# imalexlee/simple-vk-renderer

Hardware: AMD Instinct MI355X
Metric: shaded fragments/s (higher is better)
Workload: dtype f32

## Files before the change

simple-vk-renderer_amd/csrc/k_tile.hip:

```cpp
#include <hip/hip_fp16.h>

#include <hip/hip_ext.h>

#include <cstdlib>

#include "svr_launch.h"

namespace svr {

constexpr uint32_t REC_COMMON = 0x80000000u;
#ifndef SVR_PRIO_COST
#define SVR_PRIO_COST 200u
#endif
constexpr int BATCH = 64;
constexpr uint32_t SREC = 7;

constexpr float kInv255 = 0x1.010102p-8f;
constexpr float kG0 = 0x1.c51282p-2f, kG1 = -0x1.14a3a2p-2f, kG2 = 0x1.37536ap-3f, kG3 = -0x1.778474p-5f;

__device__ __forceinline__ float lod_from_rho2(float rho2) {
  uint32_t bits = f2u(rho2);
  int e = (int)(bits >> 23) - 127;
  float m = u2f((bits & 0x7fffffu) | 0x3f800000u);
  float t = m - 1.0f;
  float g = fmaf(fmaf(fmaf(kG3, t, kG2), t, kG1), t, kG0);
  float s = t * (1.0f - t);
  float l = fmaf(s, g, t);
  float lam = 0.5f * ((float)e + l);
  lam = (rho2 <= 0x1p+100f) ? lam : 50.0f;
  lam = (rho2 >= 0x1p-100f) ? lam : -50.0f;
  return lam;
}

__device__ __forceinline__ float lerpf(float a, float b, float t) { return fmaf(t, b - a, a); }

struct TexD {
  uint32_t base_off;
  uint32_t w, h, lw, lh, levels, filters;
  float min_lod, max_lod;
};

struct Taps {
  uint32_t o00, o10, o01, o11;
  float alpha, beta;
};
template <bool POW2 = false>
__device__ __forceinline__ Taps level_taps(int wl, int hl, uint32_t base, bool linear, float u, float v) {
  float U = (u - floorf(u)) * (float)wl;
  float V = (v - floorf(v)) * (float)hl;
  float Uh = U - 0.5f, Vh = V - 0.5f;
  float fu = floorf(linear ? Uh : U), fv = floorf(linear ? Vh : V);
  Taps tp;
  tp.alpha = linear ? Uh - fu : 0.0f;
  tp.beta = linear ? Vh - fv : 0.0f;
  int i0 = (int)fu, j0 = (int)fv;
  int i1 = linear ? i0 + 1 : i0, j1 = linear ? j0 + 1 : j0;
  if (POW2) {
    i0 &= wl - 1;
    i1 &= wl - 1;
    j0 &= hl - 1;
    j1 &= hl - 1;
  } else {
    if (i0 < 0) i0 += wl;
    if (i0 >= wl) i0 -= wl;
    if (i1 >= wl) i1 -= wl;
    if (j0 < 0) j0 += hl;
    if (j0 >= hl) j0 -= hl;
    if (j1 >= hl) j1 -= hl;
  }
  const uint32_t r0 = __umul24((uint32_t)j0, (uint32_t)wl), r1 = __umul24((uint32_t)j1, (uint32_t)wl);
  tp.o00 = base + (r0 + (uint32_t)i0) * 4u;
  tp.o10 = base + (r0 + (uint32_t)i1) * 4u;
  tp.o01 = base + (r1 + (uint32_t)i0) * 4u;
  tp.o11 = base + (r1 + (uint32_t)i1) * 4u;
  return tp;
}
__device__ __forceinline__ uint32_t texel(const uint8_t* arena, uint32_t off) {
  return *reinterpret_cast<const uint32_t*>(arena + off);
}
__device__ __forceinline__ float chan(uint32_t t, int c) { return (float)((t >> (8 * c)) & 0xffu) * kInv255; }
__device__ __forceinline__ float bilerp(uint32_t t00, uint32_t t10, uint32_t t01, uint32_t t11, int c, float a, float b) {
  return lerpf(lerpf(chan(t00, c), chan(t10, c), a), lerpf(chan(t01, c), chan(t11, c), a), b);
}

__device__ __forceinline__ float interp3(float a0, float da1, float da2, float b1, float b2, float r) {
  return fmaf(b2, da2, fmaf(b1, da1, a0)) * r;
}

struct FragAttr {
  float b1, b2, r, u, v, nx, ny, nz, light, cr, cg, cb, won;
};

__device__ __forceinline__ float quad_partner_x(float v) { return u2f((uint32_t)__builtin_amdgcn_mov_dpp((int)f2u(v), 0xB1, 0xf, 0xf, true)); }
__device__ __forceinline__ float quad_partner_y(float v) { return u2f((uint32_t)__builtin_amdgcn_mov_dpp((int)f2u(v), 0x128, 0xf, 0xf, true)); }
template <bool TRACE, bool COMMON = false, bool ATTR = false>
__device__ __forceinline__ float4 shade_pixel(const FrameParams& P, uint32_t rec, int px, int py, float* trace, const bool quads = false,
                                              FragAttr* fa = nullptr) {
  const TriRec* tr = P.recs + rec;
  const uint4* q4 = reinterpret_cast<const uint4*>(tr);
  const float4* f4 = reinterpret_cast<const float4*>(tr);
  const double2* d2 = reinterpret_cast<const double2*>(tr);
  uint4 hdr = q4[0];
  float4 zrow = f4[1];
  double2 c2 = d2[2], c3 = d2[3], c4 = d2[4], c5 = d2[5], c6 = d2[6];
  uint4 td = q4[7];
  float4 s0 = f4[8], s1 = f4[9], s2 = f4[10], s3 = f4[11], s4 = f4[12], s5 = f4[13], s6 = f4[14];
  uint32_t flags = hdr.w;
  float inv_area = zrow.w;
  double A1, B1, A2, B2, e1, e2;
  double C1 = c5.y, C2 = c6.x;
  A1 = c2.y; B1 = c4.x; A2 = c3.x; B2 = c4.y;
  double dx = (double)px, dy = (double)py;
  e1 = fma(A1, dx, fma(B1, dy, C1)) + ((flags & F_T1) ? 1.0 : 0.0);
  e2 = fma(A2, dx, fma(B2, dy, C2)) + ((flags & F_T2) ? 1.0 : 0.0);
  TexD t;
  t.base_off = (uint32_t)(unsigned long long)__double_as_longlong(c6.y);
  t.w = td.x & 0xffffu;
  t.h = td.x >> 16;
  t.lw = td.y & 0xffu;
  t.lh = (td.y >> 8) & 0xffu;
  t.levels = (td.y >> 16) & 0xffu;
  t.filters = td.y >> 24;
  t.min_lod = u2f(td.z);
  t.max_lod = u2f(td.w);
  float b1 = (float)e1 * inv_area, b2 = (float)e2 * inv_area;
  float q0 = s0.x, dq1 = s0.y, dq2 = s0.z;
  const float qq = fmaf(b2, dq2, fmaf(b1, dq1, q0));
  float hb1 = 0.0f, hb2 = 0.0f, vb1 = 0.0f, vb2 = 0.0f, hq = 1.0f, vq = 1.0f;
  if (!quads) {
    double sxp = (px & 1) ? -1.0 : 1.0, syp = (py & 1) ? -1.0 : 1.0;
    hb1 = (float)fma(sxp, A1, e1) * inv_area, hb2 = (float)fma(sxp, A2, e2) * inv_area;
    vb1 = (float)fma(syp, B1, e1) * inv_area, vb2 = (float)fma(syp, B2, e2) * inv_area;
    hq = fmaf(hb2, dq2, fmaf(hb1, dq1, q0)), vq = fmaf(vb2, dq2, fmaf(vb1, dq1, q0));
  }
  float r, hr = 0.0f, vr = 0.0f;
  if (COMMON && !quads) {
    rcp3_ieee(qq, hq, vq, r, hr, vr);
  } else {
    r = rcp_ieee(qq);
  }
  const uint32_t kind = COMMON ? (uint32_t)PIPE_MESH : ((flags >> F_KIND_SHIFT) & 3u);
  float cr = interp3(s1.z, s3.z, s5.z, b1, b2, r);
  float cg = interp3(s1.w, s3.w, s5.w, b1, b2, r);
  float cb = interp3(s2.x, s4.x, s6.x, b1, b2, r);
  if (ATTR) { fa->b1 = b1; fa->b2 = b2; fa->r = r; fa->won = 1.0f; }
  if (kind == PIPE_COLORED_TRIANGLE) return make_float4(cr, cg, cb, 1.0f);
  float u = interp3(s2.y, s4.y, s6.y, b1, b2, r), v = interp3(s2.z, s4.z, s6.z, b1, b2, r);
  if (ATTR) { fa->u = u; fa->v = v; }
  if (!COMMON) {
    hr = rcp_ieee(hq);
    vr = rcp_ieee(vq);
  }
  float uh, vh, uv_, vv_;
  if (quads) {
    uh = quad_partner_x(u), vh = quad_partner_x(v);
    uv_ = quad_partner_y(u), vv_ = quad_partner_y(v);
  } else {
    uh = interp3(s2.y, s4.y, s6.y, hb1, hb2, hr), vh = interp3(s2.z, s4.z, s6.z, hb1, hb2, hr);
    uv_ = interp3(s2.y, s4.y, s6.y, vb1, vb2, vr), vv_ = interp3(s2.z, s4.z, s6.z, vb1, vb2, vr);
  }
  float dudx = (px & 1) ? (u - uh) : (uh - u);
  float dvdx = (px & 1) ? (v - vh) : (vh - v);
  float dudy = (py & 1) ? (u - uv_) : (uv_ - u);
  float dvdy = (py & 1) ? (v - vv_) : (vv_ - v);
  float W0 = (float)t.w, H0 = (float)t.h;
  float mx = dudx * W0, my = dvdx * H0;
  float nx_ = dudy * W0, ny_ = dvdy * H0;
  float rho2 = fmaxf(fmaf(mx, mx, my * my), fmaf(nx_, nx_, ny_ * ny_));
  float lambda = fminf(fmaxf(lod_from_rho2(rho2), t.min_lod), t.max_lod);
  const bool linear = COMMON ? true : (((lambda <= 0.0f) ? (t.filters & 1u) : ((t.filters >> 1) & 1u)) != 0u);
  int q = (int)t.levels - 1;
  const bool mip_linear = COMMON ? true : (((t.filters >> 2) & 1u) != 0u);
  int dn = min(max((int)ceilf(lambda + 0.5f) - 1, 0), q);
  float lc = fminf(fmaxf(lambda, 0.0f), (float)q);
  float fl = floorf(lc);
  int dhi = mip_linear ? (int)fl : dn;
  float delta = mip_linear ? lc - fl : 0.0f;
  int dlo = mip_linear ? min(dhi + 1, q) : dn;
  float us = (fabsf(u) < 8388608.0f) ? u : 0.0f, vs = (fabsf(v) < 8388608.0f) ? v : 0.0f;
  const int whi = (int)max(t.w >> dhi, 1u), hhi = (int)max(t.h >> dhi, 1u);
  const uint32_t bhi = t.base_off + mip_offset(t.lw, t.lh, (uint32_t)dhi);
  Taps th = level_taps<COMMON>(whi, hhi, bhi, linear, us, vs);
  const uint8_t* tb = P.tex_arena;
  uint32_t h00 = texel(tb, th.o00), h10 = texel(tb, th.o10), h01 = texel(tb, th.o01), h11 = texel(tb, th.o11);
  const bool two_levels = __any(delta != 0.0f);
  Taps tl = th;
  uint32_t l00 = 0, l10 = 0, l01 = 0, l11 = 0;
  if (two_levels) {
    const int wlo = (int)max(t.w >> dlo, 1u), hlo = (int)max(t.h >> dlo, 1u);
    const uint32_t step = 4u << ((uint32_t)max((int)t.lw - dhi, 0) + (uint32_t)max((int)t.lh - dhi, 0));
    const uint32_t blo = dlo != dhi ? bhi + step : bhi;
    tl = level_taps<COMMON>(wlo, hlo, blo, linear, us, vs);
    l00 = texel(tb, tl.o00);
    l10 = texel(tb, tl.o10);
    l01 = texel(tb, tl.o01);
    l11 = texel(tb, tl.o11);
  }
  float4 tx;
  tx.x = bilerp(h00, h10, h01, h11, 0, th.alpha, th.beta);
  tx.y = bilerp(h00, h10, h01, h11, 1, th.alpha, th.beta);
  tx.z = bilerp(h00, h10, h01, h11, 2, th.alpha, th.beta);
  tx.w = 1.0f;
  if (two_levels) {
    tx.x = lerpf(tx.x, bilerp(l00, l10, l01, l11, 0, tl.alpha, tl.beta), delta);
    tx.y = lerpf(tx.y, bilerp(l00, l10, l01, l11, 1, tl.alpha, tl.beta), delta);
    tx.z = lerpf(tx.z, bilerp(l00, l10, l01, l11, 2, tl.alpha, tl.beta), delta);
  }
  if (TRACE) {
    trace[0] = (float)(hdr.z >> 2); trace[1] = b1; trace[2] = b2; trace[3] = r; trace[4] = u; trace[5] = v;
    trace[6] = dudx; trace[7] = dvdx; trace[8] = dudy; trace[9] = dvdy; trace[10] = lambda;
    trace[11] = tx.x; trace[12] = tx.y; trace[13] = tx.z;
    trace[26] = hb1; trace[27] = hb2; trace[28] = vb1; trace[29] = vb2; trace[30] = hr; trace[31] = vr;
  }
  if (kind == PIPE_TEX_IMAGE) {
    tx.w = bilerp(h00, h10, h01, h11, 3, th.alpha, th.beta);
    if (two_levels) tx.w = lerpf(tx.w, bilerp(l00, l10, l01, l11, 3, tl.alpha, tl.beta), delta);
    return tx;
  }
  float nx = interp3(s0.w, s2.w, s4.w, b1, b2, r);
  float ny = interp3(s1.x, s3.x, s5.x, b1, b2, r);
  float nz = interp3(s1.y, s3.y, s5.y, b1, b2, r);
  const float* L = P.scene.sunlight_direction;
  float d = fmaf(nz, L[2], fmaf(ny, L[1], nx * L[0]));
  float light = fmaxf(d, 0.1f);
  float sunw = P.scene.sunlight_color[3];
  cr = cr * tx.x;
  cg = cg * tx.y;
  cb = cb * tx.z;
  float4 o;
  o.x = fmaf(cr * light, sunw, cr * P.scene.ambient_color[0]);
  o.y = fmaf(cg * light, sunw, cg * P.scene.ambient_color[1]);
  o.z = fmaf(cb * light, sunw, cb * P.scene.ambient_color[2]);
  o.w = 1.0f;
  if (TRACE) {
    trace[15] = nx; trace[16] = ny; trace[17] = nz; trace[18] = cr; trace[19] = cg; trace[20] = cb;
    trace[21] = light; trace[22] = o.x; trace[23] = o.y; trace[24] = o.z; trace[25] = o.w;
  }
  if (ATTR) { fa->nx = nx; fa->ny = ny; fa->nz = nz; fa->light = light; fa->cr = cr; fa->cg = cg; fa->cb = cb; }
  return o;
}

template <int FMT>
struct Codec;
template <>
struct Codec<SVR_COLOR_RGBA16F> {
  typedef uint2 enc_t;
  static __device__ __forceinline__ float pin(float x) {
    asm volatile("" : "+v"(x));
    return x;
  }
  static __device__ __forceinline__ enc_t encode(float4 c) {
    c.x = pin(c.x); c.y = pin(c.y); c.z = pin(c.z); c.w = pin(c.w);
    uint32_t r = __half_as_ushort(__float2half_rn(c.x)), g = __half_as_ushort(__float2half_rn(c.y));
    uint32_t b = __half_as_ushort(__float2half_rn(c.z)), a = __half_as_ushort(__float2half_rn(c.w));
    return make_uint2(r | (g << 16), b | (a << 16));
  }
  static __device__ __forceinline__ float4 decode(enc_t e) {
    return make_float4(__half2float(__ushort_as_half((unsigned short)(e.x & 0xffffu))),
                       __half2float(__ushort_as_half((unsigned short)(e.x >> 16))),
                       __half2float(__ushort_as_half((unsigned short)(e.y & 0xffffu))),
                       __half2float(__ushort_as_half((unsigned short)(e.y >> 16))));
  }
};
template <>
struct Codec<SVR_COLOR_RGBA8> {
  typedef uint32_t enc_t;
  static __device__ __forceinline__ uint32_t un8(float f) {
    return (uint32_t)__float2int_rn(fminf(fmaxf(f, 0.0f), 1.0f) * 255.0f);
  }
  static __device__ __forceinline__ enc_t encode(float4 c) {
    return un8(c.x) | (un8(c.y) << 8) | (un8(c.z) << 16) | (un8(c.w) << 24);
  }
  static __device__ __forceinline__ float4 decode(enc_t e) {
    return make_float4(chan(e, 0), chan(e, 1), chan(e, 2), chan(e, 3));
  }
};

template <bool INSTR, bool LIST, bool HIZ>
__device__ __forceinline__ void scan_columns(const FrameParams& P, uint4* s_cov, const uint32_t* s_list, uint32_t bin_base, uint32_t n,
                                             unsigned long long* s_depth, uint32_t* s_bm, int tx0, int ty0, int ry0, int nrows,
                                             uint32_t& n_raster, uint32_t& n_hiz_bad, uint32_t& occl) {
  auto entry = [&](uint32_t i) -> uint32_t { return LIST ? (s_list[i] & 0x7fffffffu) : P.bins[bin_base + i]; };
  const uint32_t lane = threadIdx.x & 63u, wave = threadIdx.x >> 6;
  static_assert(BATCH * 8 == 512, "two pieces per thread");
  uint4 pre0 = make_uint4(0, 0, 0, 0), pre1 = pre0;
  {
    uint32_t cnt = min((uint32_t)BATCH, n);
    const bool staged = (threadIdx.x & 7u) < SREC;
    if (staged && threadIdx.x < cnt * 8u) pre0 = reinterpret_cast<const uint4*>(P.recs + entry(threadIdx.x >> 3))[threadIdx.x & 7u];
    if (staged && threadIdx.x + 256u < cnt * 8u) pre1 = reinterpret_cast<const uint4*>(P.recs + entry(32u + (threadIdx.x >> 3)))[threadIdx.x & 7u];
  }
  constexpr uint32_t SVR_HIZ_MIN = BATCH;
  constexpr uint32_t SVR_HIZ_KEEP_COLS = 192u;
  const bool hiz = HIZ && n > (uint32_t)SVR_HIZ_MIN;
  uint32_t cur = 0, hz_cols = 0, hz_batches = 0, hz_pause = 0;
  if (hiz && threadIdx.x < 32u) s_bm[threadIdx.x] = threadIdx.x < 16u ? 0u : 0xffffffffu;
  for (uint32_t b0 = 0; b0 < n; b0 += BATCH) {
    uint32_t cnt = min((uint32_t)BATCH, n - b0);
    __syncthreads();
    const bool test = hiz && b0 && hz_pause == 0u;
    if (hiz && b0 && hz_pause) hz_pause--;
    if (test) {
      cur ^= 1u;
      const uint32_t b = threadIdx.x >> 4, k = threadIdx.x & 15u;
      const uint4* c4 = reinterpret_cast<const uint4*>(s_depth + ((b & 3u) * 8u + (k >> 1)) * TILE + (b >> 2) * 8u + (k & 1u) * 4u);
      const uint4 lo = c4[0], hi = c4[1];
      atomicMin(&s_bm[cur * 16u + b], min(min(lo.y, lo.w), min(hi.y, hi.w)));
      if (threadIdx.x < 16u) s_bm[(cur ^ 1u) * 16u + threadIdx.x] = 0xffffffffu;
    }
    if (threadIdx.x < cnt * 8u && (threadIdx.x & 7u) < SREC) s_cov[(threadIdx.x >> 3) * SREC + (threadIdx.x & 7u)] = pre0;
    if (threadIdx.x + 256u < cnt * 8u && (threadIdx.x & 7u) < SREC) s_cov[(32u + (threadIdx.x >> 3)) * SREC + (threadIdx.x & 7u)] = pre1;
    __syncthreads();
    const uint4* bm4 = reinterpret_cast<const uint4*>(s_bm + cur * 16u);
    if (b0 + BATCH < n) {
      uint32_t nb = b0 + BATCH, ncnt = min((uint32_t)BATCH, n - nb);
      const bool staged = (threadIdx.x & 7u) < SREC;
      if (staged && threadIdx.x < ncnt * 8u) pre0 = reinterpret_cast<const uint4*>(P.recs + entry(nb + (threadIdx.x >> 3)))[threadIdx.x & 7u];
      if (staged && threadIdx.x + 256u < ncnt * 8u) pre1 = reinterpret_cast<const uint4*>(P.recs + entry(nb + 32u + (threadIdx.x >> 3)))[threadIdx.x & 7u];
    }
    int cx0 = 0, cw = 0;
    bool hidden = false;
    uint32_t gone = 0;
    uint32_t zb = 0, claim = 0;
    if (lane < cnt) {
      uint4 h = s_cov[lane * SREC];
      int minx = (int)(int16_t)(h.x & 0xffffu), miny = (int)(int16_t)(h.x >> 16);
      int maxx = (int)(int16_t)(h.y & 0xffffu), maxy = (int)(int16_t)(h.y >> 16);
      cx0 = max(minx, tx0);
      const int cx1 = min(maxx, tx0 + TILE - 1);
      const int cy0 = max(miny, ry0), cy1 = min(maxy, ry0 + nrows - 1);
      cw = (cx1 >= cx0 && cy1 >= cy0) ? cx1 - cx0 + 1 : 0;
      if (HIZ && cw) {
        const float4 zr = reinterpret_cast<const float4*>(s_cov)[lane * SREC + 1u];
        const float eps = (fabsf(zr.x) + fabsf(zr.y) + fabsf(zr.z)) * 0x1p-21f;
        zb = f2u(fmaxf(fmaxf(zr.x, fmaxf(zr.x + zr.y, zr.x + zr.z)) + eps, 0.0f));
        if (minx <= tx0 && maxx >= tx0 + TILE - 1 && miny <= ry0 && maxy >= ry0 + nrows - 1) {
          const double* dd = reinterpret_cast<const double*>(s_cov + lane * SREC);
          const float x0 = (float)tx0, x1 = (float)(tx0 + TILE - 1), y0 = (float)ry0, y1 = (float)(ry0 + nrows - 1);
          bool all_in = true;
          float slack = 0.0f;
          float bc[2][4];
#pragma unroll
          for (int i = 0; i < 3; i++) {
            const float A = (float)dd[4 + i], B = (float)dd[7 + i], C = (float)dd[10 + i] + ((i == 1 && (h.w & F_T1)) || (i == 2 && (h.w & F_T2)) ? 1.0f : 0.0f);
            const float M = (fabsf(C) + fmaxf(fabsf(A * x0), fabsf(A * x1)) + fmaxf(fabsf(B * y0), fabsf(B * y1))) * 0x1p-21f;
            const float e00 = fmaf(A, x0, fmaf(B, y0, C)), e10 = fmaf(A, x1, fmaf(B, y0, C));
            const float e01 = fmaf(A, x0, fmaf(B, y1, C)), e11 = fmaf(A, x1, fmaf(B, y1, C));
            all_in = all_in && fminf(fminf(e00, e10), fminf(e01, e11)) >= M + 1.0f;
            if (i) {
              bc[i - 1][0] = e00 * zr.w; bc[i - 1][1] = e10 * zr.w; bc[i - 1][2] = e01 * zr.w; bc[i - 1][3] = e11 * zr.w;
// ... 1134 lines not shown
```

simple-vk-renderer_amd/csrc/svr_api.hip:

```cpp
#include <hip/hip_runtime.h>

#include <algorithm>
#include <chrono>
#include <cmath>
#include <cstdio>
#include <cstring>
#include <deque>
#include <memory>
#include <numeric>
#include <string>
#include <vector>

#include "../../include/svr_depth.h"
#include "../../include/svr_draw_list.h"
#include "../../include/svr_attributes.h"
#include "../../include/svr_ids.h"
#include "../../include/svr_occlusion.h"
#include "../../include/svr_views.h"
#include "svr_cull.h"
#include "svr_launch.h"

using namespace svr;

namespace {
// ... 114 lines not shown
  int fmt = SVR_COLOR_RGBA16F;
  hipStream_t stream = nullptr;
  void* color_own = nullptr;
  float* depth_own = nullptr;
  void* color = nullptr;
  float* depth = nullptr;
  uint2* ids_own = nullptr;
  uint2* ids = nullptr;
  bool ids_bound = false;
  void* attr_own[4] = {};
  void* attr[4] = {};
  bool attr_bound[4] = {};
  uint32_t sx = 0, sy = 0, sw = 0, sh = 0;
  uint32_t rstride = 1, roff = 0;
  uint32_t* present_status = nullptr;

  std::vector<MeshRes> meshes;
  std::vector<ImageRes> images;
  std::vector<SvrSamplerDesc> samplers;
  std::vector<MaterialRes> materials;
  std::vector<DrawListRes> lists;
  std::vector<std::shared_ptr<PyramidMem>> pyramids;
  uint32_t occl_bound = 0;
  SvrOcclusionStats occl_stats{};
  uint64_t mesh_epoch = 0;
  uint8_t* tex_arena = nullptr;
  size_t tex_arena_cap = 0, tex_arena_top = 0;
  std::vector<std::pair<size_t, size_t>> tex_holes;
  DevBuf tex_table;
  size_t tex_slots = 0;
  DevBuf mesh_table, mat_table;
  size_t mesh_table_n = 0, mat_table_n = 0;
  int device_flatten = 0;

  struct PassSet {
    DevBuf inputs, recs, clipq, bigq, tiles, bins, pairs, flat, sorta, occl;
    hipEvent_t ev_bin = nullptr;
    hipEvent_t ev_tile = nullptr;
    bool used = false;
  };
  static const int MAX_OPS = 8;
  static const int NSETS = 4;
  PassSet sets[NSETS];
  int set_pos = 0;
  enum class OpKind { Pass, Clear, Background, Blit, Pyramid };
  enum class PassInput { Draws, Objects, List };
  struct LoggedOp {
    OpKind kind = OpKind::Pass;
    int slot = 0;
    uint32_t seq = 0;
    bool timed = false;
    FrameParams P{};
    PassInput input = PassInput::Draws;
    bool depth_only = false;
    std::vector<DrawDesc> draws;
    std::vector<SvrRenderObject> objects;
    uint32_t n_opaque_obj = 0, n_transparent_obj = 0;
    std::shared_ptr<const ListVersion> list;
    std::vector<float> viewprojs;
    std::shared_ptr<PyramidMem> pyr;
    const float* pyr_src = nullptr;
    bool flattened() const { return input != PassInput::Draws; }
    void* target = nullptr;
    int target_fmt = 0;
    uint32_t tw = 0, th = 0, y_first = 0, n_rows = 0;
    uint64_t clear_packed = 0;
    int bg_effect = 0;
    float bg_data[16] = {};
    void* blit_dst = nullptr;
    uint32_t blit_w = 0, blit_h = 0;
    int blit_fmt = 0;
    uint32_t blit_rstride = 1, blit_roff = 0, blit_row_end = 0;
    uint32_t* blit_status = nullptr;
  };
  std::deque<LoggedOp> log;
  hipEvent_t op_done[MAX_OPS] = {};
  hipEvent_t op_start[MAX_OPS] = {};
  int op_pos = 0;
  uint32_t replayed = 0;
  struct PendingClear {
    bool valid = false;
    void* target = nullptr;
    uint32_t y0 = 0, rows = 0;
    int fmt = 0;
    uint64_t packed = 0;
  } pending_clear;
  uint32_t next_seq = 1;
  uint32_t* h_failed_seq = nullptr;
  uint32_t* d_poison = nullptr;
  hipStream_t gstream = nullptr;
  hipStream_t gstream_hi = nullptr;
  hipStream_t last_g = nullptr;
  hipEvent_t ev_gswitch = nullptr;
  DevBuf d_cvt;
  uint32_t clip_cap = 0, extra_cap = 0, bin_cap = 0;
  uint32_t debug_caps = 0;
  void* h_stage[MAX_OPS] = {};
  size_t h_stage_cap[MAX_OPS] = {};
  Counters* h_counters = nullptr;
  uint32_t* h_row_cost = nullptr;
  std::vector<uint32_t> row_cost;
  uint32_t row_cost_y0 = 0, row_cost_rows = 0;

  static const int TRING = 16;
  hipEvent_t tev[TRING][5] = {};
  bool tev_used[TRING] = {};
  bool tev_all[TRING] = {};
  int tev_pos = 0;
  int kernel_timing = 0;
  double acc_ms[3] = {0, 0, 0};
  uint32_t acc_n = 0;
  FrameParams last{};
  uint32_t last_n_draws = 0;
  bool instrument = false;
  bool tile_cycles = false;
  uint32_t tuning = 0;
  int trace_x = -1, trace_y = -1;
  DevBuf d_trace, d_tile_cycles;
  SvrStats stats{};
};

namespace {

int use_device(SvrContext* ctx) {
  HIPCHK(hipSetDevice(ctx->device));
  return SVR_OK;
}

MeshRes* get_mesh(SvrContext* ctx, SvrMesh h) {
  if (h == 0 || h > ctx->meshes.size() || !ctx->meshes[h - 1].alive) return nullptr;
  return &ctx->meshes[h - 1];
}
ImageRes* get_image(SvrContext* ctx, SvrImage h) {
  if (h == 0 || h > ctx->images.size() || !ctx->images[h - 1].alive) return nullptr;
  return &ctx->images[h - 1];
}

TexBinding make_binding(const ImageRes& im, const SvrSamplerDesc& s) {
  TexBinding tb;
  std::memset(&tb, 0, sizeof(tb));
  uint32_t filters = (uint32_t)s.mag_filter | ((uint32_t)s.min_filter << 1) | ((uint32_t)s.mipmap_mode << 2);
  tb.base_off = im.arena_off;
  tb.wh = im.w | (im.h << 16);
  tb.info = im.lw | (im.lh << 8) | (im.levels << 16) | (filters << 24);
  tb.min_lod = s.min_lod;
  tb.max_lod = s.max_lod;
  return tb;
}

int finish_pending(SvrContext* ctx);

constexpr size_t ARENA_MAX = (size_t)0xffffff00u;
constexpr size_t ARENA_ALIGN = 256;

int arena_alloc(SvrContext* ctx, size_t bytes, uint32_t* off) {
  bytes = (bytes + ARENA_ALIGN - 1) & ~(ARENA_ALIGN - 1);
  for (size_t i = 0; i < ctx->tex_holes.size(); i++) {
    auto& h = ctx->tex_holes[i];
    if (h.second >= bytes) {
      *off = (uint32_t)h.first;
      h.first += bytes;
      h.second -= bytes;
      if (h.second == 0) ctx->tex_holes.erase(ctx->tex_holes.begin() + (long)i);
      return SVR_OK;
    }
  }
  if (ctx->tex_arena_top + bytes > ARENA_MAX)
    return fail(SVR_ERR_OUT_OF_MEMORY, "svr_create_image: more than 4 GiB of texels in one context");
  if (ctx->tex_arena_top + bytes > ctx->tex_arena_cap) {
    size_t want = std::max(ctx->tex_arena_cap * 2, ctx->tex_arena_top + bytes);
    want = std::min(ARENA_MAX, (want + ((size_t)64 << 20) - 1) & ~(((size_t)64 << 20) - 1));
    if (int e = finish_pending(ctx)) return e;
    HIPCHK(hipStreamSynchronize(ctx->stream));
    uint8_t* grown = nullptr;
    HIPCHK(hipMalloc((void**)&grown, want));
    if (ctx->tex_arena_top) {
      hipError_t r = hipMemcpy(grown, ctx->tex_arena, ctx->tex_arena_top, hipMemcpyDeviceToDevice);
      if (r != hipSuccess) {
        (void)hipFree(grown);
        return fail(SVR_ERR_DEVICE, std::string("hipMemcpy(texel arena): ") + hipGetErrorString(r));
      }
    }
    if (ctx->tex_arena) (void)hipFree(ctx->tex_arena);
    ctx->tex_arena = grown;
    ctx->tex_arena_cap = want;
  }
  *off = (uint32_t)ctx->tex_arena_top;
  ctx->tex_arena_top += bytes;
  return SVR_OK;
}

void arena_free(SvrContext* ctx, size_t off, size_t bytes) {
  bytes = (bytes + ARENA_ALIGN - 1) & ~(ARENA_ALIGN - 1);
  auto& holes = ctx->tex_holes;
  size_t i = 0;
  while (i < holes.size() && holes[i].first < off) i++;
  holes.insert(holes.begin() + (long)i, std::make_pair(off, bytes));
  if (i + 1 < holes.size() && holes[i].first + holes[i].second == holes[i + 1].first) {
    holes[i].second += holes[i + 1].second;
    holes.erase(holes.begin() + (long)i + 1);
  }
  if (i > 0 && holes[i - 1].first + holes[i - 1].second == holes[i].first) {
    holes[i - 1].second += holes[i].second;
    holes.erase(holes.begin() + (long)i);
  }
  if (!holes.empty() && holes.back().first + holes.back().second == ctx->tex_arena_top) {
    ctx->tex_arena_top = holes.back().first;
    holes.pop_back();
  }
}

int upload_tex_table(SvrContext* ctx, const TexBinding* scratch) {
  size_t n = ctx->materials.size() + 1;
  if (!scratch && ctx->tex_slots == n) return SVR_OK;
  std::vector<TexBinding> host(n);
  for (size_t i = 0; i < ctx->materials.size(); i++) {
    const MaterialRes& m = ctx->materials[i];
    host[i] = make_binding(ctx->images[m.image], ctx->samplers[m.sampler]);
  }
  if (scratch)
    host[n - 1] = *scratch;
  else
    std::memset(&host[n - 1], 0, sizeof(TexBinding));
  if (ctx->tex_table.cap < n * sizeof(TexBinding)) {
    HIPCHK(hipStreamSynchronize(ctx->stream));
    if (int e = ctx->tex_table.ensure(n * sizeof(TexBinding) * 2)) return e;
  }
  HIPCHK(hipMemcpyAsync(ctx->tex_table.p, host.data(), n * sizeof(TexBinding), hipMemcpyHostToDevice, ctx->stream));
  HIPCHK(hipStreamSynchronize(ctx->stream));
  ctx->tex_slots = n;
  return SVR_OK;
}

int stage_buffer(SvrContext* ctx, int slot, size_t bytes, void** out) {
  if (ctx->h_stage_cap[slot] < bytes) {
    if (ctx->h_stage[slot]) (void)hipHostFree(ctx->h_stage[slot]);
    ctx->h_stage[slot] = nullptr;
    ctx->h_stage_cap[slot] = 0;
    size_t want = bytes + bytes / 2 + 4096;
    HIPCHK(hipHostMalloc(&ctx->h_stage[slot], want, hipHostMallocDefault));
    ctx->h_stage_cap[slot] = want;
  }
  *out = ctx->h_stage[slot];
  return SVR_OK;
}

int harvest_timing(SvrContext* ctx, int slot) {
  if (!ctx->tev_used[slot]) return SVR_OK;
  HIPCHK(hipEventSynchronize(ctx->tev[slot][4]));
  const int from[3] = {0, 1, 3}, to[3] = {1, 2, 4};
  for (int k = ctx->tev_all[slot] ? 0 : 2; k < 3; k++) {
    float ms = 0.f;
    HIPCHK(hipEventElapsedTime(&ms, ctx->tev[slot][from[k]], ctx->tev[slot][to[k]]));
    ctx->acc_ms[k] += ms;
  }
  ctx->acc_n++;
  ctx->tev_used[slot] = false;
  return SVR_OK;
}

constexpr size_t TILE_HEAD_BYTES = sizeof(Counters) + (80 + ROW_COST_MAX) * sizeof(uint32_t);
static_assert(TILE_HEAD_BYTES % 16 == 0, "tile buffer head layout");

int bind_pass_buffers(SvrContext* ctx, FrameParams& P, int set_index) {
  SvrContext::PassSet& set = ctx->sets[set_index];
  if (int e = set.recs.ensure(((size_t)P.n_tris + ctx->extra_cap) * sizeof(TriRec))) return e;
  if (int e = set.clipq.ensure((size_t)ctx->clip_cap * sizeof(ClipItem))) return e;
  if (int e = set.bigq.ensure(((size_t)P.n_tris + 64) * sizeof(uint32_t))) return e;
  if (int e = set.tiles.ensure(TILE_HEAD_BYTES + ((size_t)P.n_tiles * 13 + 8 + (size_t)SPLIT_EXTRA * 8) * sizeof(uint32_t))) return e;
  if (int e = set.bins.ensure((size_t)ctx->bin_cap * sizeof(uint32_t))) return e;
  if (int e = set.pairs.ensure((size_t)ctx->bin_cap * 12)) return e;
  if (int e = set.sorta.ensure((size_t)ctx->bin_cap * 2 * sizeof(unsigned long long))) return e;
  P.recs = (TriRec*)set.recs.p;
  P.extra_cap = ctx->extra_cap;
  P.clip_queue = (ClipItem*)set.clipq.p;
  P.clip_cap = ctx->clip_cap;
  P.big_queue = (uint32_t*)set.bigq.p;
  P.counters = (Counters*)set.tiles.p;
  P.cls_count = (uint32_t*)((char*)set.tiles.p + sizeof(Counters));
  P.row_cost = P.cls_count + 80;
  P.tile_count = (uint32_t*)((char*)set.tiles.p + TILE_HEAD_BYTES);
  P.tile_offset = P.tile_count + (((size_t)P.n_tiles * 2 + 3) & ~(size_t)3);
  P.tile_info = (uint4*)(P.tile_offset + (((size_t)P.n_tiles * 2 + 3) & ~(size_t)3));
  P.tile_order = (uint32_t*)P.tile_info + ((size_t)P.n_tiles + SPLIT_EXTRA) * 8;
  P.pairs = (uint2*)set.pairs.p;
  P.pair_slot = (uint32_t*)((char*)set.pairs.p + (size_t)ctx->bin_cap * 8);
  P.bins = (uint32_t*)set.bins.p;
  P.bin_cap = ctx->bin_cap;
  P.sort_arena = (unsigned long long*)set.sorta.p;
  P.sort_cap = ctx->bin_cap * 2u;
  P.poison = ctx->d_poison;
  P.host_failed_seq = ctx->h_failed_seq;
  return SVR_OK;
}

int submit_pass(SvrContext* ctx, const SvrContext::LoggedOp& op, bool pipe) {
  FrameParams P = op.P;
  const int op_slot = op.slot;
  const std::vector<DrawDesc>& draws = op.draws;
  const bool flatten = op.flattened(), resident = op.input == SvrContext::PassInput::List;
  if (ctx->debug_caps) {
    ctx->clip_cap = std::max<uint32_t>(ctx->clip_cap, ctx->debug_caps);
    ctx->extra_cap = std::max<uint32_t>(ctx->extra_cap, ctx->debug_caps);
    ctx->bin_cap = std::max<uint32_t>(ctx->bin_cap, ctx->debug_caps);
  } else {
    ctx->clip_cap = std::max<uint32_t>(ctx->clip_cap, std::max<uint32_t>(65536u, P.n_tris / 4u));
    ctx->extra_cap = std::max<uint32_t>(ctx->extra_cap, std::max<uint32_t>(65536u, P.n_tris / 2u));
    ctx->bin_cap = std::max<uint32_t>(ctx->bin_cap, std::max<uint32_t>(1u << 22, P.n_tris * 8u));
  }
  const int set_index = ctx->set_pos;
  ctx->set_pos = (ctx->set_pos + 1) % SvrContext::NSETS;
  SvrContext::PassSet& set = ctx->sets[set_index];
  hipStream_t s = ctx->stream, g = ctx->stream;
  if (pipe) {
#ifdef SVR_AB_STAGE1_HI
    const bool hi = true;
#else
    const bool hi = P.n_tiles <= SPLIT_TILES_MAX;
#endif
    hipStream_t& slot = hi ? ctx->gstream_hi : ctx->gstream;
    if (!slot) {
      if (hi) {
        int least = 0, greatest = 0;
// ... 1848 lines not shown
```

simple-vk-renderer_amd/csrc/svr_device.h:

```cpp
#pragma once

#include <hip/hip_runtime.h>
#include <stdint.h>

#include "../../include/svr.h"

namespace svr {

constexpr int TILE = 32;
constexpr int TILE_SHIFT = 5;
constexpr int WAVE = 64;
constexpr float GUARD = 16384.0f;
constexpr uint32_t NO_REC = 0xffffffffu;
#ifndef SVR_RCP_VARIANT
#define SVR_RCP_VARIANT 1
#endif

enum PipelineKind : uint32_t { PIPE_MESH = 0, PIPE_COLORED_TRIANGLE = 1, PIPE_TEX_IMAGE = 2 };

constexpr uint32_t F_T1 = 1u;
constexpr uint32_t F_T2 = 2u;
constexpr uint32_t F_KIND_SHIFT = 4;
constexpr uint32_t F_TRANSPARENT = 256u;
constexpr uint32_t F_VIEW_SHIFT = 24;
constexpr uint32_t MAX_VIEWS = 16;

constexpr uint32_t TUNE_NO_TILE_ORDER = 1u;
constexpr uint32_t TUNE_NO_LAZY_CLEAR = 4u;
constexpr uint32_t TUNE_NO_PIPELINE = 2u;
constexpr uint32_t TUNE_NO_SPLIT = 8u;
constexpr uint32_t TUNE_HIZ = 64u;
constexpr uint32_t TUNE_NO_HIZ = 32u;
constexpr uint32_t TUNE_NO_POLL = 16u;

constexpr uint32_t SPLIT_MAX = 256;
constexpr uint32_t SPLIT_EXTRA = 4 * SPLIT_MAX;
constexpr uint32_t SPLIT_MIN_COST = 100;
constexpr uint32_t SPLIT_TILES_MAX = 4096;
constexpr uint32_t ROW_COST_MAX = 512;
#ifndef SVR_AB_TILE_SLOTS
#define SVR_AB_TILE_SLOTS 1024
#endif
constexpr uint32_t TILE_SLOTS = SVR_AB_TILE_SLOTS;
__host__ __device__ inline uint32_t tile_cost(uint32_t n_op, uint32_t n_tr) { return 40u + (n_op >> 3) + n_tr - (n_tr >> 2); }
constexpr uint32_t SPLIT_SORT_MAX = 1392;

struct DrawDesc {
  float mat[16];
  float mvp[16];
  float color_factors[4];
  const SvrVertex* vtx;
  const uint32_t* idx;
  uint32_t tri_count;
  uint32_t tri_base;
  uint32_t tex;
  uint32_t flags;
  const float* groups;
  uint32_t first_index;
  uint32_t pad;
};
static_assert(sizeof(DrawDesc) == 192 && offsetof(DrawDesc, vtx) == 144 && offsetof(DrawDesc, groups) == 176, "DrawDesc layout");
constexpr uint32_t GROUP_INDICES = 192;
__host__ __device__ inline uint32_t chunk_phase(uint32_t first_index) { return first_index % 3u == 0u ? (first_index / 3u) & 63u : 0u; }
__host__ __device__ inline uint32_t chunk_count(uint32_t first_index, uint32_t tri_count) {
  return tri_count ? (chunk_phase(first_index) + tri_count + 63u) / 64u : 0u;
}
__host__ __device__ inline uint32_t chunk_first(uint32_t first_index, uint32_t k) { return k ? 64u * k - chunk_phase(first_index) : 0u; }
__host__ __device__ inline uint32_t chunk_len(uint32_t first_index, uint32_t tri_count, uint32_t first_tri) {
  const uint32_t to_grid = 64u - ((chunk_phase(first_index) + first_tri) & 63u), left = tri_count - first_tri;
  return to_grid < left ? to_grid : left;
}
constexpr uint32_t GROUP_WORDS = 8;

struct WaveChunk {
  uint32_t draw;
  uint32_t first_tri;
};

struct TexBinding {
  uint32_t base_off;
  uint32_t pad0;
  uint32_t wh;
  uint32_t info;
  float min_lod, max_lod;
  uint32_t pad[2];
};
static_assert(sizeof(TexBinding) == 32, "TexBinding layout");

__host__ __device__ inline uint32_t mip_offset(uint32_t lw, uint32_t lh, uint32_t level) {
  const uint32_t a = lw < lh ? lw : lh, b = lw < lh ? lh : lw;
  const uint32_t l1 = level < a ? level : a;
  const uint32_t ones = l1 ? (0x55555555u >> (32u - 2u * l1)) : 0u;
  uint32_t off = ones << ((lw + lh + 4u - 2u * l1) & 31u);
  if (level > a) off += 4u * ((1u << (b - a + 1u)) - (1u << (b - level + 1u)));
  return off;
}

struct TriRec {
  int16_t minx, miny, maxx, maxy;
  uint32_t key;
  uint32_t flags;
  float z0, dz1, dz2, inv_area;
  double A[3], B[3], C[3];
  uint32_t tex_off, tex_pad;
  uint32_t tex_wh, tex_info;
  float tex_min_lod, tex_max_lod;
  float q0, dq1, dq2;
  float a0[8], da1[8], da2[8];
  float pad2;
  uint32_t object, primitive;
  float pad3[2];
};
static_assert(sizeof(TriRec) == 256, "TriRec layout");
static_assert(offsetof(TriRec, object) == 240, "TriRec layout: the ID words are piece 15's x and y");
constexpr uint32_t REC_ID_PIECE = offsetof(TriRec, object) / 16u;
static_assert(offsetof(TriRec, A) == 32 && offsetof(TriRec, tex_off) == 104 && offsetof(TriRec, tex_wh) == 112 &&
                  offsetof(TriRec, q0) == 128, "TriRec layout");

struct ClipItem {
  uint32_t draw;
  uint32_t tri;
};

struct Counters {
  uint32_t n_clip;
  uint32_t n_extra;
  uint32_t total_entries;
  uint32_t overflow;
  unsigned long long rasterized;
  unsigned long long shaded;
  unsigned long long binned;
  uint32_t n_big;
  uint32_t n_pairs;
  uint32_t n_pairs_rest;
  uint32_t sort_used;
  uint32_t n_split;
  uint32_t cost_sum;
  uint32_t flat_draws;
  uint32_t flat_tris;
  uint32_t flat_chunks;
  uint32_t flat_culled;
  uint32_t hiz_bad;
  uint32_t occl_tested;
  uint32_t occl_culled;
  uint32_t occl_tris;
};
static_assert(sizeof(Counters) == 96, "Counters layout");

struct MeshEntry {
  const SvrVertex* vtx;
  const uint32_t* idx;
  const float* groups;
  uint64_t pad;
};
struct MatEntry {
  float cf[4];
  uint32_t pass;
  uint32_t pad[3];
};

constexpr uint32_t PYR_MAX_LEVELS = 14;

struct FrameParams {
  void* color;
  float* depth;
  uint32_t W, H;
  uint32_t sx, sy, sw, sh;
  uint32_t tiles_x, tiles_y, n_tiles;
  uint32_t rstride, roff;
  const DrawDesc* draws;
  const WaveChunk* chunks;
  uint32_t n_chunks;
  uint32_t n_tris;
  TriRec* recs;
  uint32_t extra_cap;
  ClipItem* clip_queue;
  uint32_t clip_cap;
  uint32_t* big_queue;
  uint32_t* tile_count;
  uint32_t* tile_offset;
  uint32_t* cls_count;
  uint32_t* row_cost;
  uint32_t* host_row_cost;
  Counters* host_counters;
  uint32_t* host_failed_seq;
  uint32_t op_seq;
  uint32_t lazy_clear;
  uint32_t clear_lo, clear_hi;
  uint32_t flatten;
  uint32_t* poison;
  uint2* pairs;
  uint32_t* pair_slot;
  uint4* tile_info;
  unsigned long long* sort_arena;
  uint32_t sort_cap;
  uint32_t* tile_order;
  uint32_t* bins;
  uint32_t bin_cap;
  Counters* counters;
  const TexBinding* tex;
  const uint8_t* tex_arena;
  uint32_t instrument;
  int trace_x, trace_y;
  float* trace_buf;
  uint32_t* tile_cycles;
  uint32_t tuning;
  uint32_t layer_rows;
  SvrSceneData scene;
  uint2* ids;
  const uint32_t* pyr;
  uint32_t pyr_levels;
  uint32_t pyr_off[PYR_MAX_LEVELS + 1];
  uint8_t* occl_flags;
  void* attr[4];
};

constexpr uint32_t LIST_FUSED_MAX = 4096;

struct FlattenParams {
  const SvrRenderObject* objects;
  SvrRenderObject* objects_dev;
  uint32_t n_opaque, n_transparent;
  float viewproj[16];
  const MeshEntry* meshes;
  const MatEntry* materials;
  unsigned long long* keys;
  uint32_t* draw_tris;
  uint32_t* chunk_base;
  DrawDesc* draws;
  WaveChunk* chunks;
  Counters* counters;
  uint32_t ids;
  const uint32_t* obj_ids;
  uint32_t n_views;
  const float* viewprojs;
};

__device__ __forceinline__ int tile_row_y(const FrameParams& P, int ty) {
  return (int)P.sy + (ty * (int)P.rstride + (int)P.roff) * TILE;
}
__device__ __forceinline__ void local_tile_rows(const FrameParams& P, int miny, int maxy, int& l0, int& l1) {
  const int g0 = (miny - (int)P.sy) >> TILE_SHIFT, g1 = (maxy - (int)P.sy) >> TILE_SHIFT;
  l0 = g0;
  l1 = g1;
  if (P.rstride > 1u) {
    const int s = (int)P.rstride, b = g1 - (int)P.roff;
    l0 = (g0 - (int)P.roff + s - 1) / s;
    l1 = b < 0 ? -1 : b / s;
  }
}

template <bool MV>
__device__ __forceinline__ uint32_t bin_base(const FrameParams& P, uint32_t flags) {
  uint32_t b = (flags & F_TRANSPARENT) ? P.n_tiles : 0u;
  if (MV) b += (flags >> F_VIEW_SHIFT) * P.layer_rows * P.tiles_x;
  return b;
}

__device__ __forceinline__ float u2f(uint32_t u) { return __uint_as_float(u); }
__device__ __forceinline__ uint32_t f2u(float f) { return __float_as_uint(f); }

template <int VARIANT>
__device__ __forceinline__ float rcp_refined(float x) {
  float y = __builtin_amdgcn_rcpf(x);
  float r = fmaf(-x, y, 1.0f);
  y = fmaf(r, y, y);
  if (VARIANT == 2) {
    r = fmaf(-x, y, 1.0f);
    y = fmaf(r, y, y);
  }
// ... 84 lines not shown
  o.attr[5] = v.c.z;
  o.attr[6] = v.a.w;
  o.attr[7] = v.b.w;
}

__device__ __forceinline__ void colored_triangle_vert(int i, VOut& o) {
  o.clip[0] = (i == 0) ? 1.0f : (i == 1 ? -1.0f : 0.0f);
  o.clip[1] = (i == 2) ? -1.0f : 1.0f;
  o.clip[2] = 0.0f;
  o.clip[3] = 1.0f;
#pragma unroll
  for (int k = 0; k < 8; k++) o.attr[k] = 0.0f;
  o.attr[3] = (i == 0) ? 1.0f : 0.0f;
  o.attr[4] = (i == 1) ? 1.0f : 0.0f;
  o.attr[5] = (i == 2) ? 1.0f : 0.0f;
}

enum { OC_NEAR = 1, OC_FAR = 2, OC_L = 4, OC_R = 8, OC_T = 16, OC_B = 32 };
__device__ __forceinline__ int outcode(const float* c) {
  int oc = 0;
  if (c[2] > c[3]) oc |= OC_NEAR;
  if (c[2] < 0.0f) oc |= OC_FAR;
  if (c[0] < -c[3]) oc |= OC_L;
  if (c[0] > c[3]) oc |= OC_R;
  if (c[1] < -c[3]) oc |= OC_T;
  if (c[1] > c[3]) oc |= OC_B;
  return oc;
}

struct ScreenV {
  float xs, ys, zs, rw;
  bool ok;
};
__device__ __forceinline__ ScreenV to_screen(const float* c, float hw, float hh) {
  ScreenV s;
  s.rw = rcp_ieee(c[3]);
  s.xs = fmaf(c[0] * s.rw, hw, hw);
  s.ys = fmaf(c[1] * s.rw, hh, hh);
  s.zs = c[2] * s.rw;
  s.ok = (fabsf(s.xs) <= GUARD) && (fabsf(s.ys) <= GUARD);
  return s;
}

__device__ __forceinline__ void store_invalid(TriRec* rec) {
  uint4 h;
  h.x = 1u;
  h.y = 0u;
  h.z = 0u;
  h.w = 0u;
  *reinterpret_cast<uint4*>(rec) = h;
}

__device__ __forceinline__ uint32_t make_key(uint32_t seq, uint32_t draw_flags, const TexBinding& tex, bool clipped) {
  bool pow2 = (tex.wh & 0xffffu) == (1u << (tex.info & 0xffu)) && (tex.wh >> 16) == (1u << ((tex.info >> 8) & 0xffu));
  bool common = ((draw_flags >> F_KIND_SHIFT) & 3u) == PIPE_MESH && (tex.info >> 24) == 7u && pow2;
  return ((seq + 1u) << 2) | (common ? 2u : 0u) | (clipped ? 1u : 0u);
}

struct TriGeom {
  int minx, miny, maxx, maxy;
  double A[3], B[3], C[3];
};

__device__ inline bool setup_triangle(const FrameParams& P, const VOut* v0, const VOut* v1, const VOut* v2,
                                      ScreenV s0, ScreenV s1, ScreenV s2, uint32_t key, uint32_t draw_flags,
                                      const TexBinding& tex, uint4 (&rec)[16], TriGeom* geom) {
  int X0 = __float2int_rn(s0.xs * 256.0f), Y0 = __float2int_rn(s0.ys * 256.0f);
  int X1 = __float2int_rn(s1.xs * 256.0f), Y1 = __float2int_rn(s1.ys * 256.0f);
  int X2 = __float2int_rn(s2.xs * 256.0f), Y2 = __float2int_rn(s2.ys * 256.0f);
  long long area2 = (long long)(X1 - X0) * (long long)(Y2 - Y0) - (long long)(X2 - X0) * (long long)(Y1 - Y0);
  if (area2 == 0) return false;
  const bool flip = area2 < 0;
  if (flip) {
    int t;
    t = X1; X1 = X2; X2 = t;
    t = Y1; Y1 = Y2; Y2 = t;
    area2 = -area2;
  }
  const float zs1 = flip ? s2.zs : s1.zs, zs2 = flip ? s1.zs : s2.zs;
  const float rw1 = flip ? s2.rw : s1.rw, rw2 = flip ? s1.rw : s2.rw;
  int xmin = min(X0, min(X1, X2)), xmax = max(X0, max(X1, X2));
  int ymin = min(Y0, min(Y1, Y2)), ymax = max(Y0, max(Y1, Y2));
  int pminx = (xmin + 127) >> 8, pmaxx = (xmax - 128) >> 8;
  int pminy = (ymin + 127) >> 8, pmaxy = (ymax - 128) >> 8;
  pminx = max(pminx, (int)P.sx);
  pminy = max(pminy, (int)P.sy);
  pmaxx = min(pmaxx, (int)(P.sx + P.sw) - 1);
  pmaxy = min(pmaxy, (int)(P.sy + P.sh) - 1);
  if (pminx > pmaxx || pminy > pmaxy) return false;
  if (P.rstride > 1u) {
    int l0, l1;
    local_tile_rows(P, pminy, pmaxy, l0, l1);
    if (l0 > l1) return false;
  }

  int Xs[3] = {X0, X1, X2}, Ys[3] = {Y0, Y1, Y2};
  double A[3], B[3], C[3];
  uint32_t flags = draw_flags;
#pragma unroll
  for (int i = 0; i < 3; i++) {
    int a = (i + 1) % 3, b = (i + 2) % 3;
    long long dx = (long long)Xs[b] - Xs[a], dy = (long long)Ys[b] - Ys[a];
    long long Ae = -dy, Be = dx, Ce = -dx * Ys[a] + dy * Xs[a];
    bool top_left = (dy < 0) || (dy == 0 && dx > 0);
    long long Cu = Ce + 128 * (Ae + Be);
    A[i] = (double)(Ae * 256);
    B[i] = (double)(Be * 256);
    C[i] = (double)(Cu + (top_left ? 0 : -1));
    if (!top_left && i == 1) flags |= F_T1;
    if (!top_left && i == 2) flags |= F_T2;
  }
  float inv_area = rcp_ieee((float)(double)area2);
  if (geom) {
    geom->minx = pminx; geom->miny = pminy; geom->maxx = pmaxx; geom->maxy = pmaxy;
#pragma unroll
    for (int i = 0; i < 3; i++) {
      geom->A[i] = A[i]; geom->B[i] = B[i]; geom->C[i] = C[i];
    }
  }

  uint4 h;
  h.x = ((uint32_t)(uint16_t)pminx) | ((uint32_t)(uint16_t)pminy << 16);
  h.y = ((uint32_t)(uint16_t)pmaxx) | ((uint32_t)(uint16_t)pmaxy << 16);
  h.z = key;
  h.w = flags;
  rec[0] = h;
  rec[1] = make_uint4(f2u(s0.zs), f2u(zs1 - s0.zs), f2u(zs2 - s0.zs), f2u(inv_area));
  auto pack2 = [](double a, double b) {
    unsigned long long ua = (unsigned long long)__double_as_longlong(a), ub = (unsigned long long)__double_as_longlong(b);
    return make_uint4((uint32_t)ua, (uint32_t)(ua >> 32), (uint32_t)ub, (uint32_t)(ub >> 32));
  };
  rec[2] = pack2(A[0], A[1]);
  rec[3] = pack2(A[2], B[0]);
  rec[4] = pack2(B[1], B[2]);
  rec[5] = pack2(C[0], C[1]);
  {
    unsigned long long uc = (unsigned long long)__double_as_longlong(C[2]);
    rec[6] = make_uint4((uint32_t)uc, (uint32_t)(uc >> 32), tex.base_off, 0u);
  }
  rec[7] = make_uint4(tex.wh, tex.info, f2u(tex.min_lod), f2u(tex.max_lod));
  float rw0 = s0.rw;
  float sh[32];
  sh[0] = rw0;
  sh[1] = rw1 - rw0;
  sh[2] = rw2 - rw0;
#pragma unroll
  for (int k = 0; k < 8; k++) {
    const float a1 = flip ? v2->attr[k] : v1->attr[k], a2 = flip ? v1->attr[k] : v2->attr[k];
    float p0 = v0->attr[k] * rw0, p1 = a1 * rw1, p2 = a2 * rw2;
    sh[3 + k] = p0;
    sh[11 + k] = p1 - p0;
    sh[19 + k] = p2 - p0;
  }
#pragma unroll
  for (int k = 27; k < 32; k++) sh[k] = 0.0f;
#pragma unroll
  for (int k = 0; k < 8; k++) rec[8 + k] = make_uint4(f2u(sh[4 * k]), f2u(sh[4 * k + 1]), f2u(sh[4 * k + 2]), f2u(sh[4 * k + 3]));
  return true;
}

}
```

Before: 43.76 billion.

## Fetch bilinear texel pairs as 8-byte row loads and drop zrow record read

Bilinear taps now load each row's left and right texels with a single 8-byte vector load instead of two 4-byte loads. When the right tap wraps, a wave-uniform fallback refetches it separately. The texel arena gets 4 bytes of slack so the pair load cannot read past the end of the allocation. Separately, inv_area is duplicated into the previously padded shading slot, so the shader no longer needs to load record row 1 (zrow), saving one 16-byte load per fragment. The risks are extra divergence from the fix-up path and possible misaligned 8-byte loads.

```diff
diff --git a/simple-vk-renderer_amd/csrc/k_tile.hip b/simple-vk-renderer_amd/csrc/k_tile.hip
--- a/simple-vk-renderer_amd/csrc/k_tile.hip
+++ b/simple-vk-renderer_amd/csrc/k_tile.hip
@@ -41,7 +41,7 @@
 };
 
 struct Taps {
-  uint32_t o00, o10, o01, o11;
+  uint32_t o00, o01, right;
   float alpha, beta;
 };
 template <bool POW2 = false>
@@ -70,13 +70,32 @@
   }
   const uint32_t r0 = __umul24((uint32_t)j0, (uint32_t)wl), r1 = __umul24((uint32_t)j1, (uint32_t)wl);
   tp.o00 = base + (r0 + (uint32_t)i0) * 4u;
-  tp.o10 = base + (r0 + (uint32_t)i1) * 4u;
   tp.o01 = base + (r1 + (uint32_t)i0) * 4u;
-  tp.o11 = base + (r1 + (uint32_t)i1) * 4u;
+  tp.right = (uint32_t)(i1 - i0) * 4u;
   return tp;
 }
 __device__ __forceinline__ uint32_t texel(const uint8_t* arena, uint32_t off) {
   return *reinterpret_cast<const uint32_t*>(arena + off);
+}
+typedef uint32_t texel_pair_t __attribute__((ext_vector_type(2), aligned(4)));
+struct TexRow {
+  uint32_t left, right;
+};
+__device__ __forceinline__ TexRow texel_row(const uint8_t* arena, uint32_t off) {
+  const texel_pair_t p = *reinterpret_cast<const texel_pair_t*>(arena + off);
+  TexRow r;
+  r.left = p.x;
+  r.right = p.y;
+  return r;
+}
+__device__ __forceinline__ void fix_right_taps(const uint8_t* arena, const Taps& tp, TexRow& r0, TexRow& r1) {
+  const bool apart = tp.right != 4u;
+  if (__any(apart)) {
+    if (apart) {
+      r0.right = texel(arena, tp.o00 + tp.right);
+      r1.right = texel(arena, tp.o01 + tp.right);
+    }
+  }
 }
 __device__ __forceinline__ float chan(uint32_t t, int c) { return (float)((t >> (8 * c)) & 0xffu) * kInv255; }
 __device__ __forceinline__ float bilerp(uint32_t t00, uint32_t t10, uint32_t t01, uint32_t t11, int c, float a, float b) {
@@ -101,12 +120,11 @@
   const float4* f4 = reinterpret_cast<const float4*>(tr);
   const double2* d2 = reinterpret_cast<const double2*>(tr);
   uint4 hdr = q4[0];
-  float4 zrow = f4[1];
   double2 c2 = d2[2], c3 = d2[3], c4 = d2[4], c5 = d2[5], c6 = d2[6];
   uint4 td = q4[7];
   float4 s0 = f4[8], s1 = f4[9], s2 = f4[10], s3 = f4[11], s4 = f4[12], s5 = f4[13], s6 = f4[14];
   uint32_t flags = hdr.w;
-  float inv_area = zrow.w;
+  float inv_area = s6.w;
   double A1, B1, A2, B2, e1, e2;
   double C1 = c5.y, C2 = c6.x;
   A1 = c2.y; B1 = c4.x; A2 = c3.x; B2 = c4.y;
@@ -182,20 +200,22 @@
   const uint32_t bhi = t.base_off + mip_offset(t.lw, t.lh, (uint32_t)dhi);
   Taps th = level_taps<COMMON>(whi, hhi, bhi, linear, us, vs);
   const uint8_t* tb = P.tex_arena;
-  uint32_t h00 = texel(tb, th.o00), h10 = texel(tb, th.o10), h01 = texel(tb, th.o01), h11 = texel(tb, th.o11);
+  TexRow hr0 = texel_row(tb, th.o00), hr1 = texel_row(tb, th.o01);
+  fix_right_taps(tb, th, hr0, hr1);
   const bool two_levels = __any(delta != 0.0f);
   Taps tl = th;
-  uint32_t l00 = 0, l10 = 0, l01 = 0, l11 = 0;
+  TexRow lr0 = {0u, 0u}, lr1 = {0u, 0u};
   if (two_levels) {
     const int wlo = (int)max(t.w >> dlo, 1u), hlo = (int)max(t.h >> dlo, 1u);
     const uint32_t step = 4u << ((uint32_t)max((int)t.lw - dhi, 0) + (uint32_t)max((int)t.lh - dhi, 0));
     const uint32_t blo = dlo != dhi ? bhi + step : bhi;
     tl = level_taps<COMMON>(wlo, hlo, blo, linear, us, vs);
-    l00 = texel(tb, tl.o00);
-    l10 = texel(tb, tl.o10);
-    l01 = texel(tb, tl.o01);
-    l11 = texel(tb, tl.o11);
-  }
+    lr0 = texel_row(tb, tl.o00);
+    lr1 = texel_row(tb, tl.o01);
+    fix_right_taps(tb, tl, lr0, lr1);
+  }
+  const uint32_t h00 = hr0.left, h10 = hr0.right, h01 = hr1.left, h11 = hr1.right;
+  const uint32_t l00 = lr0.left, l10 = lr0.right, l01 = lr1.left, l11 = lr1.right;
   float4 tx;
   tx.x = bilerp(h00, h10, h01, h11, 0, th.alpha, th.beta);
   tx.y = bilerp(h00, h10, h01, h11, 1, th.alpha, th.beta);
diff --git a/simple-vk-renderer_amd/csrc/svr_api.hip b/simple-vk-renderer_amd/csrc/svr_api.hip
--- a/simple-vk-renderer_amd/csrc/svr_api.hip
+++ b/simple-vk-renderer_amd/csrc/svr_api.hip
@@ -290,6 +290,7 @@
 
 constexpr size_t ARENA_MAX = (size_t)0xffffff00u;
 constexpr size_t ARENA_ALIGN = 256;
+constexpr size_t ARENA_SLACK = 4;
 
 int arena_alloc(SvrContext* ctx, size_t bytes, uint32_t* off) {
   bytes = (bytes + ARENA_ALIGN - 1) & ~(ARENA_ALIGN - 1);
@@ -303,10 +304,10 @@
       return SVR_OK;
     }
   }
-  if (ctx->tex_arena_top + bytes > ARENA_MAX)
+  if (ctx->tex_arena_top + bytes + ARENA_SLACK > ARENA_MAX)
     return fail(SVR_ERR_OUT_OF_MEMORY, "svr_create_image: more than 4 GiB of texels in one context");
-  if (ctx->tex_arena_top + bytes > ctx->tex_arena_cap) {
-    size_t want = std::max(ctx->tex_arena_cap * 2, ctx->tex_arena_top + bytes);
+  if (ctx->tex_arena_top + bytes + ARENA_SLACK > ctx->tex_arena_cap) {
+    size_t want = std::max(ctx->tex_arena_cap * 2, ctx->tex_arena_top + bytes + ARENA_SLACK);
     want = std::min(ARENA_MAX, (want + ((size_t)64 << 20) - 1) & ~(((size_t)64 << 20) - 1));
     if (int e = finish_pending(ctx)) return e;
     HIPCHK(hipStreamSynchronize(ctx->stream));
diff --git a/simple-vk-renderer_amd/csrc/svr_device.h b/simple-vk-renderer_amd/csrc/svr_device.h
--- a/simple-vk-renderer_amd/csrc/svr_device.h
+++ b/simple-vk-renderer_amd/csrc/svr_device.h
@@ -107,7 +107,7 @@
   float tex_min_lod, tex_max_lod;
   float q0, dq1, dq2;
   float a0[8], da1[8], da2[8];
-  float pad2;
+  float inv_area_sh;
   uint32_t object, primitive;
   float pad3[2];
 };
@@ -115,7 +115,7 @@
 static_assert(offsetof(TriRec, object) == 240, "TriRec layout: the ID words are piece 15's x and y");
 constexpr uint32_t REC_ID_PIECE = offsetof(TriRec, object) / 16u;
 static_assert(offsetof(TriRec, A) == 32 && offsetof(TriRec, tex_off) == 104 && offsetof(TriRec, tex_wh) == 112 &&
-                  offsetof(TriRec, q0) == 128, "TriRec layout");
+                  offsetof(TriRec, q0) == 128 && offsetof(TriRec, inv_area_sh) == 236, "TriRec layout");
 
 struct ClipItem {
   uint32_t draw;
@@ -506,8 +506,9 @@
     sh[11 + k] = p1 - p0;
     sh[19 + k] = p2 - p0;
   }
-#pragma unroll
-  for (int k = 27; k < 32; k++) sh[k] = 0.0f;
+  sh[27] = inv_area;
+#pragma unroll
+  for (int k = 28; k < 32; k++) sh[k] = 0.0f;
 #pragma unroll
   for (int k = 0; k < 8; k++) rec[8 + k] = make_uint4(f2u(sh[4 * k]), f2u(sh[4 * k + 1]), f2u(sh[4 * k + 2]), f2u(sh[4 * k + 3]));
   return true;
```

Result: faster. 45.33 billion, median of 4 (+3.6%).
